# icloud-ecnu/Prophet

Hardware: AMD Instinct MI355X
Metric: GiB/s device-resident N-way gradient-bucket sum (fp32/fp16), 1/2/4/8 GPUs (higher is better)
Workload: dtype f32; 1 GPU; 8-way f32 left-fold sum of one 256 MiB bucket per GPU; n_workers=8, bucket_bytes=268435456, parallelism=key-space shard x1, kernel=byteps_reduce_sum_n

## Files before the change

prophet_amd/csrc/bpsr_api.cpp:

```cpp
#include <algorithm>
#include <atomic>
#include <cstdarg>
#include <cstdio>
#include <cstdlib>
#include <cstring>
#include <string>

#include "bpsr_api_internal.h"

namespace bpsr {

static thread_local std::string g_last_error;

int fail(int code, const char* fmt, ...) {
  char buf[512];
  va_list ap;
  va_start(ap, fmt);
  vsnprintf(buf, sizeof(buf), fmt, ap);
  va_end(ap);
  g_last_error = buf;
  return code;
}

int hip_fail(hipError_t e, const char* what) {
// ... 98 lines not shown
StageRing* stage_ring_create(size_t zero_copy_max) {
  auto* r = new StageRing();
  if (zero_copy_max) r->zero_copy_max = zero_copy_max;
  return r;
}
void stage_ring_destroy(StageRing* r) { delete r; }

static int stage_acquire(StageRing& ring, size_t bytes, StageSlot** out) {
  int dev = 0;
  hipError_t e = hipGetDevice(&dev);
  if (e != hipSuccess) return hip_fail(e, "hipGetDevice");
  StageSlot& s = ring.slots[ring.next];
  ring.next = (ring.next + 1) % kRing;
  if (s.pending) {
    note_where("ring: slot event sync");
    e = hipEventSynchronize(s.done);
    if (e != hipSuccess) return hip_fail(e, "hipEventSynchronize(stage)");
    s.pending = false;
  }
  if (s.device != dev || s.cap < bytes) {
    if (s.host) ring.retired_host.push_back(s.host);
    if (s.dev) ring.retired_dev.push_back(s.dev);
    if (s.done) (void)hipEventDestroy(s.done);
    s.host = s.host_dev = s.dev = nullptr;
    s.done = nullptr;
    note_where("ring: grow");
    const size_t cap = std::max<size_t>({bytes, 2 * s.cap, kZeroCopyTable});
    s.cap = 0;
    if ((e = hipHostMalloc(&s.host, cap, hipHostMallocMapped | hipHostMallocCoherent)) !=
        hipSuccess)
      return hip_fail(e, "hipHostMalloc(stage)");
    if ((e = hipHostGetDevicePointer(&s.host_dev, s.host, 0)) != hipSuccess)
      return hip_fail(e, "hipHostGetDevicePointer(stage)");
    if ((e = hipMalloc(&s.dev, cap)) != hipSuccess) return hip_fail(e, "hipMalloc(stage)");
    if ((e = hipEventCreateWithFlags(&s.done, hipEventDisableTiming)) != hipSuccess)
      return hip_fail(e, "hipEventCreate(stage)");
    s.cap = cap;
    s.device = dev;
  }
  *out = &s;
  return BYTEPS_REDUCE_OK;
}


int batched_with_ring(const byteps_bucket_desc* buckets, int nbuckets, int dtype, int mode,
                      hipStream_t s, StageRing* ring, hipEvent_t* done) {
  if (done) *done = nullptr;
  int rc = check_common(dtype, mode);
  if (rc) return rc;
  if (nbuckets < 0 || (nbuckets > 0 && !buckets))
    return fail(BYTEPS_REDUCE_EARGS, "bad bucket table");
  if (nbuckets == 0) return BYTEPS_REDUCE_OK;
  TableInfo ti;
  if ((rc = build_table(buckets, nbuckets, dtype, ring->table, &ti))) return rc;
  if (ti.tiles == 0) return BYTEPS_REDUCE_OK;
  StageSlot* slot = nullptr;
  if ((rc = stage_acquire(*ring, ti.bytes, &slot))) return rc;
  std::memcpy(slot->host, ring->table.data(), ti.bytes);
  hipError_t e = hipSuccess;
  const void* table = slot->host_dev;
  note_where("ring: table copy");
  if (ti.bytes > ring->zero_copy_max) {
    e = hipMemcpyAsync(slot->dev, slot->host, ti.bytes, hipMemcpyHostToDevice, s);
    if (e != hipSuccess) return hip_fail(e, "hipMemcpyAsync(batch table)");
    table = slot->dev;
  }
  note_where("ring: kernel launch");
  e = launch_batched(batch_launch(table, ti, table == slot->dev), ti.vpt, dtype, mode,
                     tuning_for_n(ti.nmax), s);
  note_where("ring: event record");
  if (e != hipSuccess) return hip_fail(e, "batched kernel launch");
  e = hipEventRecord(slot->done, s);
  if (e != hipSuccess) return hip_fail(e, "hipEventRecord(stage)");
  slot->pending = true;
  if (done) *done = slot->done;
  return BYTEPS_REDUCE_OK;
}

int fold_any_alias(void* dst, const void* const* srcs, int n, size_t len, int dtype, int mode,
                   hipStream_t s) {
  int alias = -1;
  for (int k = 0; k < n && srcs; ++k)
    if (srcs[k] == dst) alias = k;
  if (alias <= 0) return byteps_reduce_sum_n(dst, srcs, n, len, dtype, mode, s);
  int rc = check_common(dtype, mode);
  if (rc) return rc;
  if (n > kMaxSrcs)
    return fail(BYTEPS_REDUCE_EARGS, "dst aliases srcs[%d] of a %d-way fold (> %d)", alias, n,
                kMaxSrcs);
  if (len == 0) return BYTEPS_REDUCE_OK;
  for (int k = 0; k < n; ++k) {
    if (!srcs[k]) return fail(BYTEPS_REDUCE_EARGS, "null srcs[%d]", k);
    if (overlaps_partially(dst, srcs[k], len))
      return fail(BYTEPS_REDUCE_EARGS, "dst partially overlaps srcs[%d]", k);
    if (k != alias && srcs[k] == dst)
      return fail(BYTEPS_REDUCE_EARGS, "dst aliases two sources");
  }
  return fold_once(dst, srcs, n, len, dtype, mode, true, s);
}

}

using namespace bpsr;

extern "C" {

int byteps_reduce_version(void) { return BYTEPS_REDUCE_ABI_VERSION; }
// ... 322 lines not shown
```

prophet_amd/csrc/bpsr_blockq.cpp:

```cpp
#include <algorithm>
#include <cstdio>
#include <cstdlib>

#include "bpsr_api_internal.h"

namespace bpsr {

static bool epoch_released(const byteps_reduce_blockq* q, uint32_t epoch) {
  for (uint32_t r : q->rel_epoch)
    if (!epoch_reached(r, epoch)) return false;
  return true;
}

static hipError_t flush_joins(byteps_reduce_blockq* q, bool all) {
  hipError_t e = hipSuccess;
  size_t k = 0;
  for (auto& p : q->pend_join) {
    if (e == hipSuccess && (all || epoch_released(q, p.epoch))) {
      e = hipStreamWaitEvent(p.s, p.ev, 0);
      q->join_evs.push_back(p.ev);
      continue;
    }
    q->pend_join[k++] = p;
  }
// ... 64 lines not shown
                                int* pol) {
  BlockqLaunch Q{};
  Q.L = batch_launch(q->dev_table, q->ti);
  Q.flags = q->flags;
  Q.block_first = q->flags + q->nblocks;
  Q.ctl = q->ctl;
  Q.nblocks = (uint32_t)q->nblocks;
  Q.timeout_ticks = (uint64_t)(q->timeout_s * 1e3 * (double)q->clock_khz);
  Q.epoch = epoch;
  *pol = cache_pol(tu, (uint64_t)q->ti.tiles * q->ti.vpt * kBlock * 16);
  return Q;
}

static int queue_stream(byteps_reduce_blockq* q, int k, const char* what, void** stream) {
  if (!q || !stream) return fail(BYTEPS_REDUCE_EARGS, "null argument");
  hipStream_t s = nullptr;
  const hipError_t e = library_queue(q->device, q->cus, k, &s);
  if (e != hipSuccess) return hip_fail(e, what);
  *stream = reinterpret_cast<void*>(s);
  return BYTEPS_REDUCE_OK;
}

}

using namespace bpsr;

extern "C" {

int byteps_reduce_blockq_create(const byteps_bucket_desc* buckets, int nbuckets,
                                const int* block_end, int nblocks, int dtype, int mode,
                                byteps_reduce_blockq** out) {
  if (!out) return fail(BYTEPS_REDUCE_EARGS, "null block-queue out-pointer");
  *out = nullptr;
  int rc = check_common(dtype, mode);
  if (rc) return rc;
  if (nbuckets < 0 || (nbuckets > 0 && !buckets))
    return fail(BYTEPS_REDUCE_EARGS, "bad bucket table");
  if (nblocks < 1 || !block_end) return fail(BYTEPS_REDUCE_EARGS, "need >= 1 block");
  for (int k = 0; k < nblocks; ++k) {
    const int lo = k ? block_end[k - 1] : 0;
    if (block_end[k] < lo || block_end[k] > nbuckets)
      return fail(BYTEPS_REDUCE_EARGS, "block_end[%d]=%d not in [%d, %d]", k, block_end[k], lo,
                  nbuckets);
  }
  if (block_end[nblocks - 1] != nbuckets)
    return fail(BYTEPS_REDUCE_EARGS, "last block ends at %d, not at nbuckets=%d",
                block_end[nblocks - 1], nbuckets);
  std::vector<char> host;
  std::vector<uint32_t> first;
  TableInfo ti;
  int gate_occ = 2;
  if (const char* v = getenv("BPSR_BQ_GATE_OCC")) gate_occ = atoi(v);
  if (gate_occ < 1 || gate_occ > 8) gate_occ = 2;
  int force_vpt = 0;
  if (const char* v = getenv("BPSR_BQ_VPT")) force_vpt = atoi(v);
  if (force_vpt != 1 && force_vpt != 2 && force_vpt != 4) force_vpt = 0;
  if ((rc = build_table(buckets, nbuckets, dtype, host, &ti, block_end, nblocks, &first,
                        force_vpt)))
    return rc;
  auto* q = new byteps_reduce_blockq();
  q->dtype = dtype;
  q->mode = mode;
  q->nblocks = nblocks;
  q->gate_occ = gate_occ;
  q->ti = ti;
  q->rel_epoch.assign((size_t)nblocks, 0u);
  q->host_table = host;
  if (const char* v = getenv("BPSR_BQ_OWN_QUEUE")) q->own_queue = atoi(v) != 0;
  int khz = 0;
  hipError_t e = hipGetDevice(&q->device);
  if (e == hipSuccess)
    e = hipDeviceGetAttribute(&q->cus, hipDeviceAttributeMultiprocessorCount, q->device);
  if (e == hipSuccess)
    e = hipDeviceGetAttribute(&khz, hipDeviceAttributeWallClockRate, q->device);
  q->clock_khz = khz > 0 ? (uint64_t)khz : 100000;
  const size_t flag_bytes =
      (sizeof(uint32_t) * (2 * (size_t)nblocks + 1) + 255) & ~(size_t)255;
  if (e == hipSuccess && ti.tiles > 0) e = hipMalloc(&q->dev_table, ti.bytes);
  if (e == hipSuccess && ti.tiles > 0)
    e = hipMemcpy(q->dev_table, host.data(), ti.bytes, hipMemcpyHostToDevice);
  if (e == hipSuccess) e = hipMalloc(reinterpret_cast<void**>(&q->flags), flag_bytes);
  if (e == hipSuccess) e = hipMemset(q->flags, 0, sizeof(uint32_t) * nblocks);
  if (e == hipSuccess)
    e = hipMemcpy(q->flags + nblocks, first.data(), sizeof(uint32_t) * (nblocks + 1),
                  hipMemcpyHostToDevice);
  if (e == hipSuccess) e = hipMalloc(reinterpret_cast<void**>(&q->ctl), 256);
  if (e == hipSuccess) e = hipMemset(q->ctl, 0, 256);
  if (e == hipSuccess) e = hipDeviceSynchronize();
  if (e == hipSuccess)
    e = hipHostMalloc(reinterpret_cast<void**>(&q->host_err), sizeof(uint32_t));
  if (e != hipSuccess) {
    blockq_free(q);
    return hip_fail(e, "block queue setup");
  }
  *out = q;
  return BYTEPS_REDUCE_OK;
}

int byteps_reduce_blockq_config(byteps_reduce_blockq* q, int wg_per_cu, double timeout_s) {
  if (!q) return fail(BYTEPS_REDUCE_EARGS, "null block queue");
  if (q->keyed && wg_per_cu > 0)
    return fail(BYTEPS_REDUCE_EARGS, "a keyed queue has the dispatch-ordered consumer");
  if (wg_per_cu > 8) return fail(BYTEPS_REDUCE_EARGS, "wg_per_cu %d > 8", wg_per_cu);
  if (wg_per_cu > 0 && q->host_rel)
    return fail(BYTEPS_REDUCE_EARGS, "host releases need the dispatch-ordered consumer");
  if (wg_per_cu > 0 && q->overlap)
    return fail(BYTEPS_REDUCE_EARGS, "overlap needs the dispatch-ordered consumer");
  if (wg_per_cu >= 0) q->occ = wg_per_cu;
  if (timeout_s > 0) q->timeout_s = timeout_s;
// ... 258 lines not shown
```

prophet_amd/csrc/bpsr_internal.h:

```cpp
#pragma once

#include <hip/hip_runtime.h>

#include <atomic>
#include <string>
#include <stddef.h>
#include <stdint.h>

#include "bpsr/reduce.h"
#include "bpsr_error.h"

namespace bpsr {

enum : int {
  kFloat32 = 0, kFloat64 = 1, kFloat16 = 2, kUInt8 = 3,
  kInt32 = 4, kInt8 = 5, kInt64 = 6, kBFloat16 = 11
};
enum : int { kModeReference = 0, kModeAccumF32 = 1 };

constexpr int kBlock = 256;
constexpr int kMaxSrcs = 32;
constexpr uint64_t kMinTiles = 2048;

struct FoldGeom {
// ... 138 lines not shown
int batched_with_ring(const struct byteps_bucket_desc* buckets, int nbuckets, int dtype,
                      int mode, hipStream_t s, StageRing* ring, hipEvent_t* done = nullptr);

int hip_fail(hipError_t e, const char* what);

void make_geom(int dtype, size_t len, const void* dst, const void* const* srcs, int n,
               bool copy_trailing, FoldGeom* g, int* aligned);

inline int fold_grid(const FoldGeom& g, const Tuning& tu, int vpt) {
  (void)tu;
  const uint64_t tile = (uint64_t)kBlock * vpt;
  uint64_t blocks = (g.nvec + tile - 1) / tile;
  const uint64_t scalar = g.head_elems + (g.n_elems - g.tail_begin) + g.trailing_bytes;
  const uint64_t sblocks = (scalar + kBlock - 1) / kBlock;
  if (blocks == 0) blocks = sblocks < 65536 ? sblocks : 65536;
  if (blocks < 1) blocks = 1;
  return (int)blocks;
}

#define BPSR_DECLARE_LAUNCHERS(NAME)                                                      \
  hipError_t launch_fold_##NAME(const FoldArgs& a, const Tuning& tu, hipStream_t s);      \
  hipError_t launch_batched_##NAME(const BatchLaunch& L, int vpt, const Tuning& tu,      \
                                   hipStream_t s);                                        \
  hipError_t launch_blockq_##NAME(const BlockqLaunch& Q, int vpt, int pol, size_t lds,    \
                                  bool gated, hipStream_t s);
BPSR_DECLARE_LAUNCHERS(f32)
BPSR_DECLARE_LAUNCHERS(f64)
BPSR_DECLARE_LAUNCHERS(f16)
BPSR_DECLARE_LAUNCHERS(f16acc)
BPSR_DECLARE_LAUNCHERS(bf16)
BPSR_DECLARE_LAUNCHERS(bf16acc)
BPSR_DECLARE_LAUNCHERS(i8)
BPSR_DECLARE_LAUNCHERS(i32)
BPSR_DECLARE_LAUNCHERS(i64)

hipError_t launch_fold(const FoldArgs& a, int dtype, int mode, const Tuning& tu,
                       hipStream_t s);
hipError_t launch_batched(const BatchLaunch& L, int vpt, int dtype, int mode, const Tuning& tu,
                          hipStream_t s);
hipError_t launch_blockq(const BlockqLaunch& Q, int vpt, int pol, size_t lds, bool gated,
                         int dtype, int mode, hipStream_t s);
hipError_t launch_blockq_release(uint32_t* flags, uint32_t first, uint32_t count, uint32_t epoch,
                                 hipStream_t s);
hipError_t launch_key_release(uint64_t* kwords, uint32_t block, uint64_t word,
                              uint64_t* word2_at, uint64_t word2, hipStream_t s);
hipError_t read_queue_id(hipStream_t s, uint64_t* out);

inline int fold_vpt(uint64_t nvec, int vpt) {
  auto tiles = [nvec](int v) { return (nvec + (uint64_t)kBlock * v - 1) / ((uint64_t)kBlock * v); };
  while (vpt > 1 && tiles(vpt) < kMinTiles) vpt >>= 1;
  if (vpt == 2 && tiles(4) >= kMinTiles && tiles(4) < 2 * kMinTiles) vpt = 4;
  return vpt;
}
constexpr int kPolPlain = 0, kPolNt = 1, kPolWt = 2;
constexpr uint64_t kWtMaxBytes = 96ull << 20;
constexpr uint64_t kHalfTileMinBytes = 64ull << 20;
inline int cache_pol(const Tuning& tu, uint64_t bytes_per_src) {
  if (!tu.nt) return kPolPlain;
  return bytes_per_src < tu.wt_max_bytes ? kPolWt : kPolNt;
}
int fold_any_alias(void* dst, const void* const* srcs, int n, size_t len, int dtype, int mode,
                   hipStream_t s);

hipError_t launch_copy(void* dst, const void* src, size_t len, const Tuning& tu,
                       hipStream_t s);

hipError_t launch_compress_fp16(void* dst, const void* src, size_t nelem, int src_dtype,
                                const Tuning& tu, hipStream_t s);
hipError_t launch_decompress_fp16(void* dst, const void* src, size_t nelem, int dst_dtype,
                                  int divisor, const Tuning& tu, hipStream_t s);
hipError_t launch_compress_bf16(void* dst, const void* src, size_t nelem, int src_dtype,
                                const Tuning& tu, hipStream_t s);
hipError_t launch_decompress_bf16(void* dst, const void* src, size_t nelem, int dst_dtype,
                                  int divisor, const Tuning& tu, hipStream_t s);
struct CastCut {
  uint64_t head;
  uint64_t nunits;
  int aligned;
};
inline CastCut cast_cut(const void* h, const void* w, size_t nelem, int es) {
  const uintptr_t ph = (uintptr_t)h, pw = (uintptr_t)w;
  CastCut c{0, 0, (ph % 2 == 0 && pw % (uintptr_t)es == 0) ? 1 : 0};
  if (!c.aligned) return c;
  const uint64_t hh = ((16 - (ph & 15)) & 15) / 2;
  const uint64_t hw = ((16 - (pw & 15)) & 15) / (uint64_t)es;
  if (hh % (16 / (uint64_t)es) != hw || hh >= nelem) return c;
  c.nunits = (nelem - hh) / 8;
  if (c.nunits) c.head = hh;
  return c;
}

struct CastRec {
  unsigned char* wide;
  unsigned char* half;
  uint32_t kind;
  uint32_t count;
  uint32_t aligned;
  uint32_t pad;
};
static_assert(sizeof(CastRec) == 32, "CastRec layout");
constexpr uint64_t kCastElemPart = (uint64_t)kBlock * 16;
hipError_t launch_cast_plan(bool compress, const CastRec* table, uint32_t nrecords,
                            int wide_dtype, int divisor, int u, uint64_t out_bytes,
                            const Tuning& tu, hipStream_t s);
hipError_t launch_cast_plan_bf16(bool compress, const CastRec* table, uint32_t nrecords,
                                 int wide_dtype, int divisor, int u, uint64_t out_bytes,
// ... 60 lines not shown
```

prophet_amd/csrc/bpsr_kernels_impl.h:

```cpp
#pragma once

#include <hip/hip_ext.h>
#include <hip/hip_runtime.h>
#include <stdint.h>

#include "bpsr_internal.h"
#include "bpsr_ops.h"

namespace bpsr {

template <bool NT>
__device__ __forceinline__ vec16 ld16(const unsigned char* p) {
  typedef uint32_t u4 __attribute__((ext_vector_type(4)));
  if constexpr (NT) {
    return bitcast<vec16>(__builtin_nontemporal_load(reinterpret_cast<const u4*>(p)));
  } else {
    return bitcast<vec16>(*reinterpret_cast<const u4*>(p));
  }
}

template <bool NT>
__device__ __forceinline__ void st16(unsigned char* p, const vec16& v) {
  typedef uint32_t u4 __attribute__((ext_vector_type(4)));
  if constexpr (NT) {
    __builtin_nontemporal_store(bitcast<u4>(v), reinterpret_cast<u4*>(p));
  } else {
    *reinterpret_cast<u4*>(p) = bitcast<u4>(v);
  }
}

template <class E>
__device__ __forceinline__ E ld_e(const unsigned char* p, bool aligned) {
  if (aligned) return *reinterpret_cast<const E*>(p);
  E v;
  __builtin_memcpy(&v, p, sizeof(E));
  return v;
}

template <class E>
__device__ __forceinline__ void st_e(unsigned char* p, E v, bool aligned) {
  if (aligned) {
    *reinterpret_cast<E*>(p) = v;
  } else {
    __builtin_memcpy(p, &v, sizeof(E));
  }
}

constexpr int cmin(int a, int b) { return a < b ? a : b; }

using SrcPtrs = const unsigned char* const*;

template <class Op, bool NT, class XS = SrcPtrs>
__device__ __forceinline__ vec16 fold_vector_exact(const XS& srcs, int n, uint64_t off) {
  auto opaque = [](const unsigned char* p) {
    asm volatile("" : "+v"(p));
    return p;
  };
  typename Op::Acc acc = Op::init(ld16<NT>(opaque(srcs[0] + off)));
  for (int k = 1; k < n; ++k) Op::accum(acc, ld16<NT>(opaque(srcs[k] + off)));
  return Op::finish(acc);
}

template <class Op, int VPT, int NT, int NS, bool GUARD, class XS = SrcPtrs,
          class SP = const unsigned char* const*>
__device__ __forceinline__ void fold_tile_body(const SP& srcs, const XS& xsrcs, int n,
                                               unsigned char* dst, uint64_t vec_off,
                                               uint64_t v0, uint64_t nvec, int lane) {
  constexpr int NSA = NS < 0 ? -NS : NS;
  const int ns = NS > 0 ? NS : n;
  const uint64_t off0 = vec_off + (v0 + lane) * 16;
  constexpr uint64_t kStep = (uint64_t)kBlock * 16;
  constexpr int G = NSA > 0 ? cmin(NSA, 32 / VPT) : cmin(8, 32 / VPT);
  static_assert(NS >= 0 || G == NSA, "NS < 0 needs one load group");
  bool valid[VPT];
#pragma unroll
  for (int j = 0; j < VPT; ++j) valid[j] = !GUARD || (v0 + lane + (uint64_t)j * kBlock < nvec);
  typename Op::Acc acc[VPT];
  auto group = [&](int k0) __attribute__((always_inline)) {
    vec16 x[G][VPT];
#pragma unroll
    for (int g = 0; g < G; ++g) {
      if (NS > 0 || k0 + g < ns) {
        const unsigned char* base = srcs[k0 + g] + off0;
#pragma unroll
        for (int j = 0; j < VPT; ++j)
          x[g][j] = valid[j] ? ld16<(NT != 0)>(base + j * kStep) : vec16{{0, 0, 0, 0}};
      }
    }
#pragma unroll
    for (int g = 0; g < G; ++g) {
      if (NS > 0 || k0 + g < ns) {
#pragma unroll
        for (int j = 0; j < VPT; ++j) {
          if (k0 + g == 0) acc[j] = Op::init_fast(x[g][j]);
          else Op::fast(acc[j], x[g][j]);
        }
      }
    }
  };
  if constexpr (NSA > 0) {
#pragma unroll
    for (int k0 = 0; k0 < NSA; k0 += G) group(k0);
  } else {
    for (int k0 = 0; k0 < ns; k0 += G) group(k0);
  }
  bool bad = false;
#pragma unroll
  for (int j = 0; j < VPT; ++j) bad |= valid[j] && Op::has_nan(acc[j]);
#pragma unroll
  for (int j = 0; j < VPT; ++j) {
    vec16 out = Op::finish_fast(acc[j]);
    if (__builtin_expect(bad, 0)) {
      if (valid[j] && Op::has_nan(acc[j]))
        out = fold_vector_exact<Op, (NT != 0), XS>(xsrcs, ns, off0 + j * kStep);
    }
    if (valid[j]) st16<(NT != 0)>(dst + off0 + j * kStep, out);
  }
}

struct NoMid {
  __device__ __forceinline__ void operator()() const {}
};

template <class Op, int VPT, int NT, int NS, class Mid = NoMid, class XS = SrcPtrs,
          class SP = const unsigned char* const*>
__device__ __forceinline__ void fold_tile_full_buf(const SP& srcs, const XS& xsrcs, int n,
                                                   unsigned char* dst, uint64_t byte0, int lane,
                                                   const Mid& mid = Mid()) {
  constexpr int kAux = NT ? 2 : 0;
  constexpr int kStAux = NT == kPolWt ? 16 : kAux;
  constexpr int kTileBytes = kBlock * VPT * 16;
  constexpr int NSA = NS < 0 ? -NS : NS;
  constexpr int G = NSA > 0 ? cmin(NSA, 32 / VPT) : cmin(8, 32 / VPT);
  static_assert(NS >= 0 || G == NSA, "NS < 0 needs one load group");
  const int ns = NS > 0 ? NS : n;
  const int voff = lane * 16;
  typedef uint32_t u4 __attribute__((ext_vector_type(4)));
  auto rsrc = [&](const unsigned char* base) __attribute__((always_inline)) {
    return __builtin_amdgcn_make_buffer_rsrc(const_cast<unsigned char*>(base) + byte0, 0,
                                             kTileBytes, 0x00020000);
  };
  typename Op::Acc acc[VPT];
  auto group = [&](int k0) __attribute__((always_inline)) {
    vec16 x[G][VPT];
#pragma unroll
    for (int g = 0; g < G; ++g) {
      if (NS > 0 || k0 + g < ns) {
        const auto r = rsrc(srcs[k0 + g]);
#pragma unroll
        for (int j = 0; j < VPT; ++j)
          x[g][j] = bitcast<vec16>(__builtin_amdgcn_raw_buffer_load_b128(r, voff + j * kBlock * 16,
                                                                         0, kAux));
      }
    }
#pragma unroll
    for (int g = 0; g < G; ++g) {
      if (NS > 0 || k0 + g < ns) {
#pragma unroll
        for (int j = 0; j < VPT; ++j) {
          if (k0 + g == 0) acc[j] = Op::init_fast(x[g][j]);
          else Op::fast(acc[j], x[g][j]);
        }
      }
    }
  };
  if constexpr (NSA > 0) {
#pragma unroll
    for (int k0 = 0; k0 < NSA; k0 += G) group(k0);
  } else {
    for (int k0 = 0; k0 < ns; k0 += G) group(k0);
  }
  mid();
  bool bad = false;
#pragma unroll
  for (int j = 0; j < VPT; ++j) bad = bad || Op::has_nan(acc[j]);
  const auto rd = __builtin_amdgcn_make_buffer_rsrc(dst + byte0, 0, kTileBytes, 0x00020000);
#pragma unroll
  for (int j = 0; j < VPT; ++j) {
    vec16 out = Op::finish_fast(acc[j]);
    if (__builtin_expect(bad, 0)) {
      if (Op::has_nan(acc[j]))
        out = fold_vector_exact<Op, (NT != 0), XS>(xsrcs, ns, byte0 + voff + j * kBlock * 16);
    }
    __builtin_amdgcn_raw_buffer_store_b128(bitcast<u4>(out), rd, voff + j * kBlock * 16, 0, kStAux);
  }
}

template <class Op, int VPT, int NT, int NS>
__device__ __forceinline__ void fold_tile(const unsigned char* const* srcs, int n,
                                          unsigned char* dst, uint64_t vec_off, uint64_t v0,
                                          uint64_t nvec, int lane) {
  if (v0 + (uint64_t)kBlock * VPT <= nvec)
    fold_tile_full_buf<Op, VPT, NT, NS>(srcs, srcs, n, dst, vec_off + v0 * 16, lane);
  else
    fold_tile_body<Op, VPT, NT, NS, true>(srcs, srcs, n, dst, vec_off, v0, nvec, lane);
}

template <class Op, class XS = SrcPtrs>
__device__ __forceinline__ void fold_elements(const XS& srcs, int n,
                                              unsigned char* dst, const FoldGeom& g,
                                              bool aligned, uint64_t t, uint64_t stride) {
  using E = typename Op::E;
  const uint64_t n_head = g.head_elems;
  const uint64_t n_tail = g.n_elems - g.tail_begin;
  const uint64_t n_scalar = n_head + n_tail;
  for (uint64_t s = t; s < n_scalar; s += stride) {
    const uint64_t e = s < n_head ? s : g.tail_begin + (s - n_head);
    const bool tail = e >= g.tail_sem_from;
    const uint64_t off = e * sizeof(E);
    typename Op::EAcc acc{};
    for (int k0 = 0; k0 < n; k0 += 8) {
      E x[8];
#pragma unroll
      for (int q = 0; q < 8; ++q)
        if (k0 + q < n) x[q] = ld_e<E>(srcs[k0 + q] + off, aligned);
#pragma unroll
      for (int q = 0; q < 8; ++q) {
        if (k0 + q < n) {
          if (k0 + q == 0) acc = Op::init_e(x[q], tail);
          else Op::accum_e(acc, x[q], tail);
        }
      }
    }
    st_e<E>(dst + off, Op::finish_e(acc, tail), aligned);
  }
  if (g.copy_trailing) {
    const uint64_t tb = g.n_elems * sizeof(E);
    for (uint64_t b = t; b < g.trailing_bytes; b += stride) dst[tb + b] = srcs[0][tb + b];
  }
}

template <int NS>
__device__ __forceinline__ void pin_args(const FoldArgs& a) {
  if constexpr (NS == 8) {
    asm volatile("" ::"s"(a.srcs[0]), "s"(a.srcs[1]), "s"(a.srcs[2]), "s"(a.srcs[3]),
                 "s"(a.srcs[4]), "s"(a.srcs[5]), "s"(a.srcs[6]), "s"(a.srcs[7]), "s"(a.dst),
                 "s"(a.g.nvec), "s"(a.g.vec_off), "s"(a.grid));
  } else if constexpr (NS == 2) {
    asm volatile("" ::"s"(a.srcs[0]), "s"(a.srcs[1]), "s"(a.dst), "s"(a.g.nvec),
                 "s"(a.g.vec_off), "s"(a.grid));
  } else if constexpr (NS == 16) {
    asm volatile("" ::"s"(a.srcs[0]), "s"(a.srcs[1]), "s"(a.srcs[2]), "s"(a.srcs[3]),
                 "s"(a.srcs[4]), "s"(a.srcs[5]), "s"(a.srcs[6]), "s"(a.srcs[7]),
                 "s"(a.srcs[8]), "s"(a.srcs[9]), "s"(a.srcs[10]), "s"(a.srcs[11]),
                 "s"(a.srcs[12]), "s"(a.srcs[13]), "s"(a.srcs[14]), "s"(a.srcs[15]),
                 "s"(a.dst), "s"(a.g.nvec), "s"(a.g.vec_off), "s"(a.grid));
  } else {
    asm volatile("" ::"s"(a.dst), "s"(a.g.nvec), "s"(a.g.vec_off), "s"(a.grid));
  }
}

template <class Op, int VPT, int NT, int NS>
__global__ __launch_bounds__(kBlock) void fold_kernel(FoldArgs a) {
  pin_args<NS>(a);
  const uint64_t tile_vecs = (uint64_t)kBlock * VPT;
  const uint64_t full = a.g.nvec / tile_vecs;
  const bool partial = full * tile_vecs < a.g.nvec;
  const uint64_t bid = blockIdx.x;
  const int elem_mode = a.g.nvec == 0 ? 2 : (bid == 0 ? 1 : 0);
  const uint64_t tile = partial ? (bid == 0 ? full : bid - 1) : bid;
  if (tile < full)
    fold_tile_full_buf<Op, VPT, NT, NS>(a.srcs, a.srcs, a.n, a.dst,
                                        a.g.vec_off + tile * tile_vecs * 16, threadIdx.x);
  else if (tile * tile_vecs < a.g.nvec)
    fold_tile_body<Op, VPT, NT, NS, true>(a.srcs, a.srcs, a.n, a.dst, a.g.vec_off,
                                          tile * tile_vecs, a.g.nvec, threadIdx.x);
  if (elem_mode == 2)
    fold_elements<Op>(a.srcs, a.n, a.dst, a.g, a.aligned != 0,
                      (uint64_t)blockIdx.x * kBlock + threadIdx.x, (uint64_t)a.grid * kBlock);
  else if (elem_mode == 1)
    fold_elements<Op>(a.srcs, a.n, a.dst, a.g, a.aligned != 0, threadIdx.x, kBlock);
}

struct RecRegs {
  unsigned char* dst;
  uint32_t kind, n, a, b, c;
  const unsigned char* p[8];
};

template <class Op, int VPT, int NT, class Mid = NoMid>
__device__ __forceinline__ void run_record(const RecRegs& r, const unsigned char* const* msrcs,
                                           const BatchEntry* entries, const Mid& mid = Mid()) {
  if (r.kind == kTileElem) {
    const BatchEntry& e = entries[r.b];
    fold_elements<Op>(e.srcs, e.n, e.dst, e.g, e.aligned != 0,
                      (uint64_t)r.a * kBlock + threadIdx.x, (uint64_t)r.c * kBlock);
    mid();
  } else if (r.n <= 8) {
    if (r.kind == kTileFull) {
      fold_tile_full_buf<Op, VPT, NT, -8>(r.p, msrcs, (int)r.n, r.dst, 0, threadIdx.x, mid);
    } else {
      fold_tile_body<Op, VPT, NT, -8, true>(r.p, msrcs, (int)r.n, r.dst, 0, 0, r.a, threadIdx.x);
      mid();
    }
  } else {
    if (r.kind == kTileFull) {
      fold_tile_full_buf<Op, VPT, NT, 0>(msrcs, msrcs, (int)r.n, r.dst, 0, threadIdx.x, mid);
    } else {
      fold_tile_body<Op, VPT, NT, 0, true>(msrcs, msrcs, (int)r.n, r.dst, 0, 0, r.a,
                                           threadIdx.x);
      mid();
    }
  }
}

__device__ __forceinline__ RecRegs load_record(const unsigned char* rec) {
  const TileHead& h = *reinterpret_cast<const TileHead*>(rec);
  const unsigned char* const* msrcs =
      reinterpret_cast<const unsigned char* const*>(rec + kTileHeadBytes);
  RecRegs r;
  r.dst = h.dst;
  r.kind = h.kind;
  r.n = h.n;
  r.a = h.a;
  r.b = h.b;
  r.c = h.c;
#pragma unroll
  for (int k = 0; k < 8; ++k) r.p[k] = msrcs[k];
  asm volatile("" ::"s"(r.dst), "s"(r.kind), "s"(r.n), "s"(r.a), "s"(r.p[0]), "s"(r.p[1]),
               "s"(r.p[2]), "s"(r.p[3]), "s"(r.p[4]), "s"(r.p[5]), "s"(r.p[6]), "s"(r.p[7]));
  return r;
}

constexpr int kRecWords = (kTileHeadBytes + 8 * 8) / 4;
__device__ __forceinline__ RecRegs regs_from_words(const uint32_t* w) {
  uint32_t v[kRecWords];
#pragma unroll
  for (int k = 0; k < kRecWords; ++k) v[k] = __builtin_amdgcn_readfirstlane(w[k]);
  auto ptr = [&](int k) {
    return reinterpret_cast<unsigned char*>(((uint64_t)v[k + 1] << 32) | v[k]);
  };
  RecRegs r;
  r.dst = ptr(0);
  r.kind = v[2];
  r.n = v[3];
  r.a = v[4];
  r.b = v[5];
  r.c = v[6];
#pragma unroll
  for (int k = 0; k < 8; ++k) r.p[k] = ptr(8 + 2 * k);
  return r;
}

__device__ __forceinline__ uint32_t prefetch_record(const BatchLaunch& L, uint64_t b) {
  uint32_t v = 0;
  const uint64_t t = b + L.pf_ahead;
  if (L.pf_ahead != 0 && threadIdx.x < 2 && t < L.tiles) {
    const uint32_t* p = reinterpret_cast<const uint32_t*>(L.recs + t * L.rec_stride);
    v = p[threadIdx.x == 0 ? 0 : L.rec_stride / 4 - 1];
  }
  return v;
}
__device__ __forceinline__ void keep_prefetch(uint32_t v) { asm volatile("" ::"v"(v)); }
// ... 256 lines not shown
  if (threadIdx.x == 0) kt[0] = wall_clock64();
#endif
  const unsigned char* rec = Q.L.recs + (uint64_t)t * Q.L.rec_stride;
  const RecRegs r = load_record(rec);
  const uint32_t blk = reinterpret_cast<const TileHead*>(rec)->block;
  const uint32_t pf = prefetch_record(Q.L, t);
  const uint64_t* wp = Q.kwords + (uint64_t)blk * kKeyWordStride;
  uint64_t w = ld_agent64(wp);
  if ((uint32_t)w != Q.epoch) {
    const uint64_t t0 = wall_clock64();
    for (;;) {
      __builtin_amdgcn_s_sleep(8);
      w = ld_agent64(wp);
      if ((uint32_t)w == Q.epoch) break;
      if (ld_err(Q)) return;
      if (wall_clock64() - t0 > Q.timeout_ticks) {
        __hip_atomic_store(&Q.ctl->err, 1u, __ATOMIC_RELAXED, __HIP_MEMORY_SCOPE_AGENT);
        return;
      }
    }
    __builtin_amdgcn_fence(__ATOMIC_ACQUIRE, "agent");
  }
#ifdef BPSR_KEYED_TRACE
  if (threadIdx.x == 0) kt[1] = wall_clock64();
#endif
  const uint32_t perm = (uint32_t)(w >> 32);
  if (perm == kKeySkip) {
    keep_prefetch(pf);
    key_tile_done<NT>(Q, blk, true);
    return;
  }
  if (Q.wide) {
    const uint64_t* hp = Q.kwords + (uint64_t)(Q.nblocks + blk) * kKeyWordStride;
    uint64_t hi = ld_agent64(hp);
    const uint64_t t0 = wall_clock64();
    while ((uint32_t)hi != Q.epoch) {
      __builtin_amdgcn_s_sleep(2);
      hi = ld_agent64(hp);
      if (wall_clock64() - t0 > Q.timeout_ticks) {
        __hip_atomic_store(&Q.ctl->err, 1u, __ATOMIC_RELAXED, __HIP_MEMORY_SCOPE_AGENT);
        return;
      }
    }
    const uint64_t perm64 = ((hi >> 32) << 32) | perm;
    const unsigned char* const* m =
        reinterpret_cast<const unsigned char* const*>(rec + kTileHeadBytes);
    const PermSrcs16 ps{m, perm64};
    if (r.kind == kTileElem) {
      const BatchEntry& e = Q.L.entries[r.b];
      fold_elements<Op, PermSrcs16>(PermSrcs16{e.srcs, perm64}, e.n, e.dst, e.g,
                                    e.aligned != 0, (uint64_t)r.a * kBlock + threadIdx.x,
                                    (uint64_t)r.c * kBlock);
    } else if (r.kind == kTileFull) {
      fold_tile_full_buf<Op, VPT, NT, 0, NoMid, PermSrcs16>(ps, ps, (int)r.n, r.dst, 0,
                                                            threadIdx.x);
    } else {
      fold_tile_body<Op, VPT, NT, 0, true, PermSrcs16>(ps, ps, (int)r.n, r.dst, 0, 0, r.a,
                                                        threadIdx.x);
    }
    keep_prefetch(pf);
    key_tile_done<NT>(Q, blk, r.kind == kTileFull && NT == kPolWt);
    return;
  }
  const unsigned char* q[8];
#pragma unroll
  for (int m = 0; m < 8; ++m) {
    const uint32_t wk = (perm >> (4 * m)) & 7u;
    const unsigned char* v = r.p[0];
#pragma unroll
    for (int k = 1; k < 8; ++k) v = wk == (uint32_t)k ? r.p[k] : v;
    q[m] = v;
  }
  const PermSrcs xs{reinterpret_cast<const unsigned char* const*>(rec + kTileHeadBytes), perm};
  if (r.kind == kTileElem) {
    const BatchEntry& e = Q.L.entries[r.b];
    fold_elements<Op, PermSrcs>(PermSrcs{e.srcs, perm}, e.n, e.dst, e.g, e.aligned != 0,
                                (uint64_t)r.a * kBlock + threadIdx.x, (uint64_t)r.c * kBlock);
  } else if (r.kind == kTileFull) {
    fold_tile_full_buf<Op, VPT, NT, -8, NoMid, PermSrcs>(q, xs, (int)r.n, r.dst, 0,
                                                         threadIdx.x);
  } else {
    fold_tile_body<Op, VPT, NT, -8, true, PermSrcs>(q, xs, (int)r.n, r.dst, 0, 0, r.a,
                                                     threadIdx.x);
  }
  keep_prefetch(pf);
#ifdef BPSR_KEYED_TRACE
  if (threadIdx.x == 0) kt[2] = wall_clock64();
#endif
  key_tile_done<NT>(Q, blk, r.kind == kTileFull && NT == kPolWt);
#ifdef BPSR_KEYED_TRACE
  if (threadIdx.x == 0) kt[3] = wall_clock64();
#endif
}


template <class K, class A>
static hipError_t launch_with_stop(K kernel, uint32_t grid, size_t lds, hipStream_t s,
                                   hipEvent_t stop, const A& arg) {
  if (stop)
    hipExtLaunchKernelGGL(kernel, dim3(grid), dim3(kBlock), (uint32_t)lds, s, nullptr, stop, 0, arg);
  else
    hipLaunchKernelGGL(kernel, dim3(grid), dim3(kBlock), lds, s, arg);
  return hipGetLastError();
}

template <class Op, int VPT, int NT, int NS>
static hipError_t launch_fold_ns(const FoldArgs& a, const Tuning& tu, hipStream_t s) {
  static KernelAttr attr;
  const hipError_t lds_ok =
      allow_lds(attr, reinterpret_cast<const void*>(&fold_kernel<Op, VPT, NT, NS>));
  if (lds_ok != hipSuccess) return lds_ok;
  FoldArgs b = a;
  b.grid = (uint32_t)fold_grid(a.g, tu, VPT);
  hipLaunchKernelGGL((fold_kernel<Op, VPT, NT, NS>), dim3(b.grid), dim3(kBlock),
                     occ_lds_bytes(launch_occ(tu, b.grid, false)), s, b);
  return hipGetLastError();
}

template <class Op, int VPT, int NT>
static hipError_t launch_fold_vpt(const FoldArgs& a, const Tuning& tu, hipStream_t s) {
  switch (a.n) {
    case 2: return launch_fold_ns<Op, VPT, NT, 2>(a, tu, s);
    case 8: return launch_fold_ns<Op, VPT, NT, 8>(a, tu, s);
    case 16: return launch_fold_ns<Op, VPT, NT, 16>(a, tu, s);
    default: return launch_fold_ns<Op, VPT, NT, 0>(a, tu, s);
  }
}

template <class Op, int NT>
static hipError_t launch_fold_pol(const FoldArgs& a, int vpt, const Tuning& tu, hipStream_t s) {
  switch (vpt) {
    case 1: return launch_fold_vpt<Op, 1, NT>(a, tu, s);
    case 4: return launch_fold_vpt<Op, 4, NT>(a, tu, s);
    default: return launch_fold_vpt<Op, 2, NT>(a, tu, s);
  }
}

template <class Op>
static hipError_t launch_fold_op(const FoldArgs& a, const Tuning& tu, hipStream_t s) {
  int vpt = fold_vpt(a.g.nvec, tu.vpt);
  const int pol = cache_pol(tu, a.g.nvec * 16);
  Tuning t = tu;
  if (pol == kPolWt && vpt == 2 && tu.occ == 1 && a.g.nvec * 16 >= kHalfTileMinBytes) {
    vpt = 1;
    t.occ = 2;
  }
  switch (pol) {
    case kPolNt: return launch_fold_pol<Op, kPolNt>(a, vpt, t, s);
    case kPolWt: return launch_fold_pol<Op, kPolWt>(a, vpt, t, s);
    default: return launch_fold_pol<Op, kPolPlain>(a, vpt, t, s);
  }
}

template <class Op, int VPT>
static hipError_t launch_batched_vpt(const BatchLaunch& L, const Tuning& tu, hipStream_t s) {
  static KernelAttr attr[3];
  const void* k[3] = {reinterpret_cast<const void*>(&batched_kernel<Op, VPT, kPolPlain>),
                      reinterpret_cast<const void*>(&batched_kernel<Op, VPT, kPolNt>),
                      reinterpret_cast<const void*>(&batched_kernel<Op, VPT, kPolWt>)};
  note_where("batched: allow_lds");
  for (int i = 0; i < 3; ++i) {
    const hipError_t ok = allow_lds(attr[i], k[i]);
    if (ok != hipSuccess) return ok;
  }
  note_where("batched: launch");
  if (L.tiles == 0) return hipSuccess;
  const size_t lds = occ_lds_bytes(launch_occ(tu, L.tiles, true));
  switch (cache_pol(tu, (uint64_t)L.tiles * VPT * kBlock * 16)) {
    case kPolNt: return launch_with_stop(batched_kernel<Op, VPT, kPolNt>, L.tiles, lds, s, L.stop, L);
    case kPolWt: return launch_with_stop(batched_kernel<Op, VPT, kPolWt>, L.tiles, lds, s, L.stop, L);
    default: return launch_with_stop(batched_kernel<Op, VPT, kPolPlain>, L.tiles, lds, s, L.stop, L);
  }
}

template <class Op>
static hipError_t launch_batched_op(const BatchLaunch& L, int vpt, const Tuning& tu,
                                    hipStream_t s) {
  switch (vpt) {
    case 1: return launch_batched_vpt<Op, 1>(L, tu, s);
    case 4: return launch_batched_vpt<Op, 4>(L, tu, s);
    default: return launch_batched_vpt<Op, 2>(L, tu, s);
  }
}

template <class Op, int VPT, int NT>
static hipError_t launch_blockq_k(const BlockqLaunch& Q, size_t lds, bool gated, hipStream_t s) {
  if (Q.keyed) {
    static KernelAttr attr_k;
    const hipError_t okk =
        allow_lds(attr_k, reinterpret_cast<const void*>(&blockq_key_kernel<Op, VPT, NT>));
    if (okk != hipSuccess) return okk;
    return launch_with_stop(blockq_key_kernel<Op, VPT, NT>, Q.grid, lds, s, Q.L.stop, Q);
  }
  if (gated) {
    static KernelAttr attr_g;
    const hipError_t okg =
        allow_lds(attr_g, reinterpret_cast<const void*>(&blockq_gate_kernel<Op, VPT, NT>));
    if (okg != hipSuccess) return okg;
    return launch_with_stop(blockq_gate_kernel<Op, VPT, NT>, Q.grid, lds, s, Q.L.stop, Q);
  }
  static KernelAttr attr_p;
  const hipError_t ok = allow_lds(attr_p, reinterpret_cast<const void*>(&blockq_kernel<Op, VPT, NT>),
                                  (int)kLdsPerCU - 256);
  if (ok != hipSuccess) return ok;
  return launch_with_stop(blockq_kernel<Op, VPT, NT>, Q.grid, lds, s, Q.L.stop, Q);
}

template <class Op, int VPT>
static hipError_t launch_blockq_vpt(const BlockqLaunch& Q, int pol, size_t lds, bool gated,
                                    hipStream_t s) {
  switch (pol) {
    case kPolNt: return launch_blockq_k<Op, VPT, kPolNt>(Q, lds, gated, s);
    case kPolWt: return launch_blockq_k<Op, VPT, kPolWt>(Q, lds, gated, s);
    default: return launch_blockq_k<Op, VPT, kPolPlain>(Q, lds, gated, s);
  }
}

template <class Op>
static hipError_t launch_blockq_op(const BlockqLaunch& Q, int vpt, int pol, size_t lds,
                                   bool gated, hipStream_t s) {
  if (Q.grid == 0) return hipSuccess;
  switch (vpt) {
    case 1: return launch_blockq_vpt<Op, 1>(Q, pol, lds, gated, s);
    case 4: return launch_blockq_vpt<Op, 4>(Q, pol, lds, gated, s);
    default: return launch_blockq_vpt<Op, 2>(Q, pol, lds, gated, s);
  }
}

}

#define BPSR_DEFINE_LAUNCHERS(NAME, OP)                                                   \
  namespace bpsr {                                                                        \
  hipError_t launch_fold_##NAME(const FoldArgs& a, const Tuning& tu, hipStream_t s) {     \
    return launch_fold_op<OP>(a, tu, s);                                                  \
  }                                                                                       \
  hipError_t launch_batched_##NAME(const BatchLaunch& L, int vpt, const Tuning& tu,      \
                                   hipStream_t s) {                                       \
    return launch_batched_op<OP>(L, vpt, tu, s);                                          \
  }                                                                                       \
  hipError_t launch_blockq_##NAME(const BlockqLaunch& Q, int vpt, int pol, size_t lds,    \
                                  bool gated, hipStream_t s) {                            \
    return launch_blockq_op<OP>(Q, vpt, pol, lds, gated, s);                               \
  }                                                                                       \
  }
```

prophet_amd/csrc/bpsr_table.cpp:

```cpp
#include <algorithm>
#include <cstdlib>
#include <cstring>

#include "bpsr_api_internal.h"

namespace bpsr {

int elem_size(int dtype) {
  switch (dtype) {
    case kInt8: case kUInt8: return 1;
    case kFloat16: case kBFloat16: return 2;
    case kInt32: case kFloat32: return 4;
    case kInt64: case kFloat64: return 8;
    default: return 0;
  }
}

void make_geom(int dtype, size_t len, const void* dst, const void* const* srcs, int n,
               bool copy_trailing, FoldGeom* g, int* aligned) {
  const uint64_t es = (uint64_t)elem_size(dtype);
  std::memset(g, 0, sizeof(*g));
  g->n_elems = len / es;
  g->trailing_bytes = len % es;
  g->copy_trailing = (copy_trailing && g->trailing_bytes) ? 1u : 0u;
  const uintptr_t d = (uintptr_t)dst;
  bool elem_al = (d % es) == 0, co = true;
  for (int k = 0; k < n; ++k) {
    const uintptr_t s = (uintptr_t)srcs[k];
    elem_al = elem_al && (s % es) == 0;
    co = co && ((s & 15u) == (d & 15u));
  }
  *aligned = elem_al ? 1 : 0;
  const uint64_t vec_end = dtype == kFloat16 ? (g->n_elems / 8) * 8 : g->n_elems;
  g->tail_sem_from = dtype == kFloat16 ? vec_end : g->n_elems;
  if (elem_al && co) {
    uint64_t head = ((16u - (d & 15u)) & 15u) / es;
    if (head > g->n_elems) head = g->n_elems;
    g->head_elems = head;
    g->vec_off = head * es;
    g->nvec = vec_end > head ? ((vec_end - head) * es) / 16 : 0;
    g->tail_begin = head + g->nvec * 16 / es;
  } else {
    g->head_elems = 0;
    g->vec_off = 0;
    g->nvec = 0;
    g->tail_begin = 0;
  }
}

constexpr uint64_t kElemPart = (uint64_t)kBlock * 16;

int build_table(const byteps_bucket_desc* buckets, int nbuckets, int dtype, std::vector<char>& out,
                TableInfo* ti, const int* block_end, int nblocks,
                std::vector<uint32_t>* block_first, int force_vpt) {
  std::vector<BatchEntry> tab;
  std::vector<int> tab_block;
  tab.reserve(nbuckets);
  int blk = 0;
  uint64_t vecs = 0;
  int nmax = 1;
  for (int i = 0; i < nbuckets; ++i) {
    const byteps_bucket_desc& b = buckets[i];
    if (b.n < 1 || b.n > kMaxSrcs)
      return fail(BYTEPS_REDUCE_EARGS, "bucket %d: n=%d outside [1, %d]", i, b.n, kMaxSrcs);
    while (block_end && blk < nblocks && i >= block_end[blk]) ++blk;
    if (b.len == 0) continue;
    if (!b.dst) return fail(BYTEPS_REDUCE_EARGS, "bucket %d: null dst", i);
    for (int k = 0; k < b.n; ++k) {
      if (!b.srcs[k]) return fail(BYTEPS_REDUCE_EARGS, "bucket %d: null srcs[%d]", i, k);
      if (overlaps_partially(b.dst, b.srcs[k], b.len) || (k > 0 && b.srcs[k] == b.dst))
        return fail(BYTEPS_REDUCE_EARGS, "bucket %d: dst overlaps srcs[%d]", i, k);
    }
    BatchEntry e;
    std::memset(&e, 0, sizeof(e));
    for (int k = 0; k < b.n; ++k) e.srcs[k] = static_cast<const unsigned char*>(b.srcs[k]);
    e.dst = static_cast<unsigned char*>(b.dst);
    e.n = b.n;
    make_geom(dtype, b.len, b.dst, b.srcs, b.n, b.dst != b.srcs[0], &e.g, &e.aligned);
    vecs += e.g.nvec;
    nmax = std::max(nmax, b.n);
    tab.push_back(e);
    tab_block.push_back(blk);
  }
  const int vpt = force_vpt ? force_vpt : fold_vpt(vecs, launch_tuning_for_n(nmax).vpt);
  const uint64_t tile_vecs = (uint64_t)kBlock * vpt;
  auto elem_parts = [](const BatchEntry& e) -> uint64_t {
    const uint64_t n_scalar = e.g.head_elems + (e.g.n_elems - e.g.tail_begin);
    const bool trailing = e.g.copy_trailing && e.g.trailing_bytes > 0;
    if (n_scalar == 0 && !trailing) return 0;
    const uint64_t p = (n_scalar + kElemPart - 1) / kElemPart;
    return std::min<uint64_t>(std::max<uint64_t>(p, 1), 65536);
  };
  uint64_t tiles = 0;
  for (auto& e : tab) tiles += elem_parts(e) + (e.g.nvec + tile_vecs - 1) / tile_vecs;
  if (tiles >= (1ull << 32) / kBlock) return fail(BYTEPS_REDUCE_EARGS, "batch too large");
  const uint32_t stride = tile_rec_stride(nmax);
  const size_t recs_off = ((sizeof(BatchEntry) * tab.size()) + 255) & ~(size_t)255;
  out.assign(recs_off + (size_t)stride * tiles, 0);
  if (!tab.empty()) std::memcpy(out.data(), tab.data(), sizeof(BatchEntry) * tab.size());
  char* rec = out.data() + recs_off;
  uint32_t cur_block = 0;
  auto put = [&](unsigned char* dst, uint32_t kind, const BatchEntry& e, uint32_t a, uint32_t b,
                 uint32_t c, uint64_t byte0) {
    TileHead h;
    std::memset(&h, 0, sizeof(h));
    h.dst = dst + byte0;
    h.kind = kind;
    h.n = (uint32_t)e.n;
    h.a = a;
    h.b = b;
    h.c = c;
    h.block = cur_block;
    std::memcpy(rec, &h, sizeof(h));
    const unsigned char** p = reinterpret_cast<const unsigned char**>(rec + kTileHeadBytes);
    for (int k = 0; k < e.n; ++k) p[k] = e.srcs[k] + byte0;
    rec += stride;
  };
  auto emit = [&](size_t b0, size_t b1) {
    for (size_t b = b0; b < b1; ++b) {
      const uint64_t parts = elem_parts(tab[b]);
      for (uint64_t q = 0; q < parts; ++q)
        put(tab[b].dst, kTileElem, tab[b], (uint32_t)q, (uint32_t)b, (uint32_t)parts, 0);
    }
    for (size_t b = b0; b < b1; ++b) {
      const BatchEntry& e = tab[b];
      for (uint64_t v0 = 0; v0 < e.g.nvec; v0 += tile_vecs) {
        const uint64_t left = e.g.nvec - v0;
        const bool full = left >= tile_vecs;
        put(e.dst, full ? kTileFull : kTilePartial, e, full ? 0u : (uint32_t)left, (uint32_t)b,
            0, e.g.vec_off + v0 * 16);
      }
    }
  };
  char* const rec0 = rec;
  if (!block_end) {
    emit(0, tab.size());
  } else {
    block_first->assign((size_t)nblocks + 1, 0);
    size_t b0 = 0;
    for (int k = 0; k < nblocks; ++k) {
      size_t b1 = b0;
      while (b1 < tab.size() && tab_block[b1] == k) ++b1;
      (*block_first)[k] = (uint32_t)((rec - rec0) / stride);
      cur_block = (uint32_t)k;
      emit(b0, b1);
      b0 = b1;
    }
    (*block_first)[nblocks] = (uint32_t)tiles;
  }
  ti->vpt = vpt;
  ti->nmax = nmax;
  ti->live = (int)tab.size();
  ti->tiles = (uint32_t)tiles;
  ti->rec_stride = stride;
  ti->recs_off = recs_off;
  ti->bytes = out.size();
  return BYTEPS_REDUCE_OK;
}

BatchLaunch batch_launch(const void* dev_table, const TableInfo& ti, bool in_hbm) {
  BatchLaunch L;
  L.entries = static_cast<const BatchEntry*>(dev_table);
  L.recs = static_cast<const unsigned char*>(dev_table) + ti.recs_off;
  L.rec_stride = ti.rec_stride;
  L.tiles = ti.tiles;
  static const uint32_t ahead = [] {
    const char* v = getenv("BPSR_REC_PREFETCH");
    const long x = v ? atol(v) : (long)kPrefetchAhead;
    return x > 0 ? (uint32_t)((x + 7) & ~7L) : 0u;
  }();
  L.pf_ahead = in_hbm ? ahead : 0u;
  L.stop = nullptr;
  return L;
}

}
// ... 1 lines not shown
```

Baseline: 5491 GiB/s.

## Add 8-vector-per-thread tiles with a half-size drain tail in batch table

Result: no change. 5497 GiB/s, median of 2 (+0.1%).

```diff
diff --git a/prophet_amd/csrc/bpsr_api.cpp b/prophet_amd/csrc/bpsr_api.cpp
--- a/prophet_amd/csrc/bpsr_api.cpp
+++ b/prophet_amd/csrc/bpsr_api.cpp
@@ -174,7 +174,9 @@
     return fail(BYTEPS_REDUCE_EARGS, "bad bucket table");
   if (nbuckets == 0) return BYTEPS_REDUCE_OK;
   TableInfo ti;
-  if ((rc = build_table(buckets, nbuckets, dtype, ring->table, &ti))) return rc;
+  if ((rc = build_table(buckets, nbuckets, dtype, ring->table, &ti, nullptr, 0, nullptr,
+                        env_table_vpt() == 8 ? 8 : 0)))
+    return rc;
   if (ti.tiles == 0) return BYTEPS_REDUCE_OK;
   StageSlot* slot = nullptr;
   if ((rc = stage_acquire(*ring, ti.bytes, &slot))) return rc;
diff --git a/prophet_amd/csrc/bpsr_blockq.cpp b/prophet_amd/csrc/bpsr_blockq.cpp
--- a/prophet_amd/csrc/bpsr_blockq.cpp
+++ b/prophet_amd/csrc/bpsr_blockq.cpp
@@ -140,9 +140,7 @@
   int gate_occ = 2;
   if (const char* v = getenv("BPSR_BQ_GATE_OCC")) gate_occ = atoi(v);
   if (gate_occ < 1 || gate_occ > 8) gate_occ = 2;
-  int force_vpt = 0;
-  if (const char* v = getenv("BPSR_BQ_VPT")) force_vpt = atoi(v);
-  if (force_vpt != 1 && force_vpt != 2 && force_vpt != 4) force_vpt = 0;
+  const int force_vpt = env_table_vpt();
   if ((rc = build_table(buckets, nbuckets, dtype, host, &ti, block_end, nblocks, &first,
                         force_vpt)))
     return rc;
diff --git a/prophet_amd/csrc/bpsr_internal.h b/prophet_amd/csrc/bpsr_internal.h
--- a/prophet_amd/csrc/bpsr_internal.h
+++ b/prophet_amd/csrc/bpsr_internal.h
@@ -214,6 +214,13 @@
   if (vpt == 2 && tiles(4) >= kMinTiles && tiles(4) < 2 * kMinTiles) vpt = 4;
   return vpt;
 }
+inline int table_vpt(uint64_t nvec, int vpt) {
+  const int v = fold_vpt(nvec, vpt);
+  if (v == 4 && vpt < 4 && nvec / ((uint64_t)kBlock * 8) >= kMinTiles / 2) return 8;
+  return v;
+}
+constexpr uint64_t kDrainTiles = 512;
+int env_table_vpt();
 constexpr int kPolPlain = 0, kPolNt = 1, kPolWt = 2;
 constexpr uint64_t kWtMaxBytes = 96ull << 20;
 constexpr uint64_t kHalfTileMinBytes = 64ull << 20;
diff --git a/prophet_amd/csrc/bpsr_kernels_impl.h b/prophet_amd/csrc/bpsr_kernels_impl.h
--- a/prophet_amd/csrc/bpsr_kernels_impl.h
+++ b/prophet_amd/csrc/bpsr_kernels_impl.h
@@ -71,7 +71,7 @@
   const uint64_t off0 = vec_off + (v0 + lane) * 16;
   constexpr uint64_t kStep = (uint64_t)kBlock * 16;
   constexpr int G = NSA > 0 ? cmin(NSA, 32 / VPT) : cmin(8, 32 / VPT);
-  static_assert(NS >= 0 || G == NSA, "NS < 0 needs one load group");
+  static_assert(NS >= 0 || NSA % G == 0, "NS < 0 needs whole load groups");
   bool valid[VPT];
 #pragma unroll
   for (int j = 0; j < VPT; ++j) valid[j] = !GUARD || (v0 + lane + (uint64_t)j * kBlock < nvec);
@@ -131,8 +131,9 @@
   constexpr int kStAux = NT == kPolWt ? 16 : kAux;
   constexpr int kTileBytes = kBlock * VPT * 16;
   constexpr int NSA = NS < 0 ? -NS : NS;
-  constexpr int G = NSA > 0 ? cmin(NSA, 32 / VPT) : cmin(8, 32 / VPT);
-  static_assert(NS >= 0 || G == NSA, "NS < 0 needs one load group");
+  constexpr int kLoads = (VPT == 8 && sizeof(typename Op::Acc) > sizeof(vec16)) ? 16 : 32;
+  constexpr int G = NSA > 0 ? cmin(NSA, kLoads / VPT) : cmin(8, kLoads / VPT);
+  static_assert(NS >= 0 || NSA % G == 0, "NS < 0 needs whole load groups");
   const int ns = NS > 0 ? NS : n;
   const int voff = lane * 16;
   typedef uint32_t u4 __attribute__((ext_vector_type(4)));
@@ -184,6 +185,22 @@
     }
     __builtin_amdgcn_raw_buffer_store_b128(bitcast<u4>(out), rd, voff + j * kBlock * 16, 0, kStAux);
   }
+}
+
+constexpr int small_vpt(int vpt) { return vpt == 8 ? 4 : vpt; }
+
+template <class Op, int VPT, int NT, int NS, class Mid = NoMid, class XS = SrcPtrs,
+          class SP = const unsigned char* const*>
+__device__ __forceinline__ void fold_tile_full_sized(const SP& srcs, const XS& xsrcs, int n,
+                                                     unsigned char* dst, bool big, int lane,
+                                                     const Mid& mid = Mid()) {
+  if constexpr (VPT == 8) {
+    if (big) {
+      fold_tile_full_buf<Op, 8, NT, NS, Mid, XS, SP>(srcs, xsrcs, n, dst, 0, lane, mid);
+      return;
+    }
+  }
+  fold_tile_full_buf<Op, small_vpt(VPT), NT, NS, Mid, XS, SP>(srcs, xsrcs, n, dst, 0, lane, mid);
 }
 
 template <class Op, int VPT, int NT, int NS>
@@ -288,17 +305,20 @@
     mid();
   } else if (r.n <= 8) {
     if (r.kind == kTileFull) {
-      fold_tile_full_buf<Op, VPT, NT, -8>(r.p, msrcs, (int)r.n, r.dst, 0, threadIdx.x, mid);
+      fold_tile_full_sized<Op, VPT, NT, -8>(r.p, msrcs, (int)r.n, r.dst, r.c == 8, threadIdx.x,
+                                            mid);
     } else {
-      fold_tile_body<Op, VPT, NT, -8, true>(r.p, msrcs, (int)r.n, r.dst, 0, 0, r.a, threadIdx.x);
+      fold_tile_body<Op, small_vpt(VPT), NT, -8, true>(r.p, msrcs, (int)r.n, r.dst, 0, 0, r.a,
+                                                       threadIdx.x);
       mid();
     }
   } else {
     if (r.kind == kTileFull) {
-      fold_tile_full_buf<Op, VPT, NT, 0>(msrcs, msrcs, (int)r.n, r.dst, 0, threadIdx.x, mid);
+      fold_tile_full_sized<Op, VPT, NT, 0>(msrcs, msrcs, (int)r.n, r.dst, r.c == 8, threadIdx.x,
+                                           mid);
     } else {
-      fold_tile_body<Op, VPT, NT, 0, true>(msrcs, msrcs, (int)r.n, r.dst, 0, 0, r.a,
-                                           threadIdx.x);
+      fold_tile_body<Op, small_vpt(VPT), NT, 0, true>(msrcs, msrcs, (int)r.n, r.dst, 0, 0, r.a,
+                                                      threadIdx.x);
       mid();
     }
   }
@@ -661,11 +681,11 @@
                                     e.aligned != 0, (uint64_t)r.a * kBlock + threadIdx.x,
                                     (uint64_t)r.c * kBlock);
     } else if (r.kind == kTileFull) {
-      fold_tile_full_buf<Op, VPT, NT, 0, NoMid, PermSrcs16>(ps, ps, (int)r.n, r.dst, 0,
-                                                            threadIdx.x);
+      fold_tile_full_sized<Op, VPT, NT, 0, NoMid, PermSrcs16>(ps, ps, (int)r.n, r.dst, r.c == 8,
+                                                              threadIdx.x);
     } else {
-      fold_tile_body<Op, VPT, NT, 0, true, PermSrcs16>(ps, ps, (int)r.n, r.dst, 0, 0, r.a,
-                                                        threadIdx.x);
+      fold_tile_body<Op, small_vpt(VPT), NT, 0, true, PermSrcs16>(ps, ps, (int)r.n, r.dst, 0, 0,
+                                                                   r.a, threadIdx.x);
     }
     keep_prefetch(pf);
     key_tile_done<NT>(Q, blk, r.kind == kTileFull && NT == kPolWt);
@@ -686,11 +706,11 @@
     fold_elements<Op, PermSrcs>(PermSrcs{e.srcs, perm}, e.n, e.dst, e.g, e.aligned != 0,
                                 (uint64_t)r.a * kBlock + threadIdx.x, (uint64_t)r.c * kBlock);
   } else if (r.kind == kTileFull) {
-    fold_tile_full_buf<Op, VPT, NT, -8, NoMid, PermSrcs>(q, xs, (int)r.n, r.dst, 0,
-                                                         threadIdx.x);
+    fold_tile_full_sized<Op, VPT, NT, -8, NoMid, PermSrcs>(q, xs, (int)r.n, r.dst, r.c == 8,
+                                                           threadIdx.x);
   } else {
-    fold_tile_body<Op, VPT, NT, -8, true, PermSrcs>(q, xs, (int)r.n, r.dst, 0, 0, r.a,
-                                                     threadIdx.x);
+    fold_tile_body<Op, small_vpt(VPT), NT, -8, true, PermSrcs>(q, xs, (int)r.n, r.dst, 0, 0, r.a,
+                                                                threadIdx.x);
   }
   keep_prefetch(pf);
 #ifdef BPSR_KEYED_TRACE
@@ -788,6 +808,7 @@
   switch (vpt) {
     case 1: return launch_batched_vpt<Op, 1>(L, tu, s);
     case 4: return launch_batched_vpt<Op, 4>(L, tu, s);
+    case 8: return launch_batched_vpt<Op, 8>(L, tu, s);
     default: return launch_batched_vpt<Op, 2>(L, tu, s);
   }
 }
@@ -832,6 +853,7 @@
   switch (vpt) {
     case 1: return launch_blockq_vpt<Op, 1>(Q, pol, lds, gated, s);
     case 4: return launch_blockq_vpt<Op, 4>(Q, pol, lds, gated, s);
+    case 8: return launch_blockq_vpt<Op, 8>(Q, pol, lds, gated, s);
     default: return launch_blockq_vpt<Op, 2>(Q, pol, lds, gated, s);
   }
 }
diff --git a/prophet_amd/csrc/bpsr_table.cpp b/prophet_amd/csrc/bpsr_table.cpp
--- a/prophet_amd/csrc/bpsr_table.cpp
+++ b/prophet_amd/csrc/bpsr_table.cpp
@@ -46,6 +46,12 @@
     g->nvec = 0;
     g->tail_begin = 0;
   }
+}
+
+int env_table_vpt() {
+  const char* v = getenv("BPSR_BQ_VPT");
+  const int x = v ? atoi(v) : 0;
+  return x == 1 || x == 2 || x == 4 || x == 8 ? x : 0;
 }
 
 constexpr uint64_t kElemPart = (uint64_t)kBlock * 16;
@@ -82,8 +88,15 @@
     tab.push_back(e);
     tab_block.push_back(blk);
   }
-  const int vpt = force_vpt ? force_vpt : fold_vpt(vecs, launch_tuning_for_n(nmax).vpt);
+  const int vpt = force_vpt ? force_vpt : table_vpt(vecs, launch_tuning_for_n(nmax).vpt);
   const uint64_t tile_vecs = (uint64_t)kBlock * vpt;
+  const bool mixed = vpt == 8;
+  const uint64_t half_vecs = tile_vecs / 2;
+  auto vec_tiles = [&](const BatchEntry& e) -> uint64_t {
+    if (!mixed) return (e.g.nvec + tile_vecs - 1) / tile_vecs;
+    const uint64_t rem = e.g.nvec % tile_vecs;
+    return e.g.nvec / tile_vecs + (rem >= half_vecs) + (rem % half_vecs != 0);
+  };
   auto elem_parts = [](const BatchEntry& e) -> uint64_t {
     const uint64_t n_scalar = e.g.head_elems + (e.g.n_elems - e.g.tail_begin);
     const bool trailing = e.g.copy_trailing && e.g.trailing_bytes > 0;
@@ -92,7 +105,12 @@
     return std::min<uint64_t>(std::max<uint64_t>(p, 1), 65536);
   };
   uint64_t tiles = 0;
-  for (auto& e : tab) tiles += elem_parts(e) + (e.g.nvec + tile_vecs - 1) / tile_vecs;
+  for (auto& e : tab) tiles += elem_parts(e) + vec_tiles(e);
+  uint64_t total32 = 0, seen32 = 0;
+  if (mixed)
+    for (auto& e : tab) total32 += e.g.nvec / tile_vecs;
+  const uint64_t drain32 = std::min<uint64_t>(kDrainTiles / 2, total32 / 4);
+  tiles += drain32;
   if (tiles >= (1ull << 32) / kBlock) return fail(BYTEPS_REDUCE_EARGS, "batch too large");
   const uint32_t stride = tile_rec_stride(nmax);
   const size_t recs_off = ((sizeof(BatchEntry) * tab.size()) + 255) & ~(size_t)255;
@@ -122,6 +140,30 @@
       for (uint64_t q = 0; q < parts; ++q)
         put(tab[b].dst, kTileElem, tab[b], (uint32_t)q, (uint32_t)b, (uint32_t)parts, 0);
     }
+    if (mixed) {
+      for (size_t b = b0; b < b1; ++b) {
+        const BatchEntry& e = tab[b];
+        const uint64_t left = e.g.nvec % half_vecs;
+        if (left)
+          put(e.dst, kTilePartial, e, (uint32_t)left, (uint32_t)b, 0,
+              e.g.vec_off + (e.g.nvec - left) * 16);
+      }
+      for (size_t b = b0; b < b1; ++b) {
+        const BatchEntry& e = tab[b];
+        uint64_t v0 = 0;
+        for (; v0 + tile_vecs <= e.g.nvec; v0 += tile_vecs) {
+          if (seen32++ < total32 - drain32) {
+            put(e.dst, kTileFull, e, 0, (uint32_t)b, 8, e.g.vec_off + v0 * 16);
+          } else {
+            put(e.dst, kTileFull, e, 0, (uint32_t)b, 4, e.g.vec_off + v0 * 16);
+            put(e.dst, kTileFull, e, 0, (uint32_t)b, 4, e.g.vec_off + (v0 + half_vecs) * 16);
+          }
+        }
+        if (v0 + half_vecs <= e.g.nvec)
+          put(e.dst, kTileFull, e, 0, (uint32_t)b, 4, e.g.vec_off + v0 * 16);
+      }
+      return;
+    }
     for (size_t b = b0; b < b1; ++b) {
       const BatchEntry& e = tab[b];
       for (uint64_t v0 = 0; v0 < e.g.nvec; v0 += tile_vecs) {
```
